# donahowe/TheaterGen

Hardware: AMD Instinct MI355X
Metric: 512px 50-step char images/sec (node), CMIGBench 4-turn story (higher is better)
Workload: dtype bf16; 1 GPU; SD-1.5 512x512, 4-turn story x 2 characters = 8 char images per step per GPU, 50 DDIM steps, CFG 7.5, IP-Adapter 77+4 tokens scale 0.4, bf16, random-init weights; plan=sd15, char_batch=8, cfg_batch=16, streams=1, ddim_steps=50, parallelism=dialogue-sharded x1 (RCCL broadcast + all_gather only)

## Files before the change

theatergen_amd/build.py:

```python
import hashlib
import os
import subprocess
import sys
from concurrent.futures import ThreadPoolExecutor

HERE = os.path.dirname(os.path.abspath(__file__))
CSRC = os.path.join(HERE, "csrc")
OBJ = os.path.join(CSRC, "_build")
LIBDIR = os.path.join(HERE, "lib")
LIB = os.path.join(LIBDIR, "libtheatergen_hip.so")
HEADER = os.path.join(os.path.dirname(HERE), "include", "theatergen_hip.h")
ARCH = "gfx950"
FLAGS = ["--offload-arch=" + ARCH, "-O3", "-std=c++17", "-fPIC",
         "-Wno-unused-result"]


EXTRA_FLAGS = {"tg_rowchain.hip": ["-mllvm", "-pragma-unroll-threshold=1000000"]}

BUILD_INFO = os.path.join(LIBDIR, "build_info.json")


def _write_build_info():
    import json

    def git(*a):
        try:
            return subprocess.run(["git", "-C", HERE] + list(a), capture_output=True, text=True).stdout.strip()
        except OSError:
            return ""
    info = {"commit": git("rev-parse", "--short", "HEAD"), "csrc_dirty": bool(git("status", "--porcelain", "--", CSRC, HEADER)),
            "sources_sha256": _digest(sources() + sorted(os.path.join(CSRC, f) for f in os.listdir(CSRC) if f.endswith(".h")) + [HEADER])[:16]}
    with open(BUILD_INFO, "w") as f:
        json.dump(info, f)


def _hipcc():
    for c in (os.environ.get("HIPCC"), "/opt/rocm/bin/hipcc", "hipcc"):
        if c and (os.path.isabs(c) and os.path.exists(c) or not os.path.isabs(c)):
            return c
    return "hipcc"


def _digest(paths):
    h = hashlib.sha256()
    for p in paths:
        with open(p, "rb") as f:
            h.update(f.read())
    h.update(" ".join(FLAGS).encode())
    for p_ in paths:
        h.update(" ".join(EXTRA_FLAGS.get(os.path.basename(p_), [])).encode())
    return h.hexdigest()


def sources():
    return sorted(os.path.join(CSRC, f) for f in os.listdir(CSRC) if f.endswith(".hip"))


def build(force=False, verbose=True, check_gate=False):
    os.makedirs(OBJ, exist_ok=True)
    os.makedirs(LIBDIR, exist_ok=True)
    srcs = sources()
    deps = [os.path.join(CSRC, f) for f in os.listdir(CSRC) if f.endswith(".h")] + [HEADER]
    hipcc = _hipcc()
    todo = []
    objs = []
    for s in srcs:
        o = os.path.join(OBJ, os.path.basename(s)[:-4] + ".o")
        stamp = o + ".sha"
        dg = _digest([s] + deps)
        objs.append(o)
        if force or not os.path.exists(o) or not os.path.exists(o + ".res") or not os.path.exists(stamp) or open(stamp).read() != dg:
            todo.append((s, o, stamp, dg))

    def compile_one(job):
        s, o, stamp, dg = job
        cmd = [hipcc] + FLAGS + EXTRA_FLAGS.get(os.path.basename(s), []) + ["-Rpass-analysis=kernel-resource-usage", "-c", s, "-o", o]
        if verbose:
            print("[build]", " ".join(cmd), flush=True)
        r = subprocess.run(cmd, capture_output=True, text=True)
        if r.returncode != 0:
            raise RuntimeError(f"hipcc failed for {s}:\n{r.stdout}\n{r.stderr}")
        with open(o + ".res", "w") as f:
            f.write(r.stderr)
        with open(stamp, "w") as f:
            f.write(dg)

    if todo:
        with ThreadPoolExecutor(max_workers=min(8, len(todo))) as ex:
            list(ex.map(compile_one, todo))
    if todo or not os.path.exists(LIB):
        cmd = [hipcc, "--offload-arch=" + ARCH, "-shared", "-fPIC", "-o", LIB] + objs
        if verbose:
            print("[build]", " ".join(cmd), flush=True)
        r = subprocess.run(cmd, capture_output=True, text=True)
        if r.returncode != 0:
            raise RuntimeError(f"link failed:\n{r.stdout}\n{r.stderr}")
    if todo or not os.path.exists(BUILD_INFO):
        _write_build_info()
    if check_gate or os.environ.get("TG_BUILD_GATE") == "1":
        write_resources(check=True, verbose=verbose, report=False)
    return LIB


RESOURCES_JSON = os.path.join(os.path.dirname(HERE), "profiles", "r6_kernel_resources.json")
HOT_GATES = [
    ("attention_kernel<bf16,48,64,true,true,false,false>", 0, 128),
    ("attention_kernel<f16,48,64,true,true,false,false>", 0, 128),
    ("attention_kernel<", 0, 256),
    ("gemm_glds_kernel<", 0, 256),
    ("conv_halo_kernel<", 0, 256),
    ("conv_slab_kernel<", 320, 256),
    ("bt_gemm_kernel<", 132, 256),
    ("rc_xattn_kernel<", 0, 256),
    ("rc_ff_kernel<", 0, 256),
    ("rc_front_kernel<", 0, 216),
    ("rc_linear_kernel<", 0, 256),
    ("skinny_gemm_kernel<", 0, 256),
    ("attn_bwd_kernel<", 0, 224),
    ("pp_gemm_kernel<bf16,2,", 0, 256),
    ("pp_gemm_kernel<f16,2,", 0, 256),
    ("pp_gemm_kernel<bf16,0,0>", 0, 256),
    ("pp_gemm_kernel<f16,0,0>", 0, 256),
    ("pp_gemm_kernel<", 256, 256),
    ("conv_in_mfma_kernel<", 0, 256),
    ("conv_out_mfma_kernel<", 0, 128),
]


def _pretty(sym):
    import re
    m = re.match(r"_ZN12_GLOBAL__N_1(\d+)", sym) or re.match(r"_Z(\d+)", sym)
    if not m:
        return sym
    n = int(m.group(1))
    base, rest = sym[m.end():m.end() + n], sym[m.end() + n:]
    if not rest.startswith("I"):
        return base
    args, i = [], 1
    while i < len(rest) and rest[i] != "E":
        if rest.startswith("DF16b", i):
            args.append("bf16"); i += 5
        elif rest.startswith("DF16_", i):
            args.append("f16"); i += 5
        elif rest[i] == "L":
            j = rest.index("E", i)
            tok = rest[i + 1:j]
            if tok[0] == "b":
                args.append("true" if tok[1:] == "1" else "false")
            else:
                args.append(re.sub(r"^[a-z]n?", lambda mm: "-" if mm.group(0).endswith("n") and len(mm.group(0)) > 1 else "", tok))
            i = j + 1
        elif rest[i] in "fidjlmb":
            args.append({"f": "float", "i": "int", "d": "double", "j": "unsigned", "l": "long", "m": "unsigned long", "b": "bool"}[rest[i]]); i += 1
        else:
            args.append("?" + rest[i:i + 12]); break
    return base + "<" + ",".join(args) + ">"


def _demangle(names):
    return [_pretty(n) for n in names]


def kernel_resources(verbose=True):
    import re
    keys = {"VGPRs": "vgprs", "AGPRs": "agprs", "ScratchSize [bytes/lane]": "scratch", "Occupancy [waves/SIMD]": "occupancy",
            "SGPRs Spill": "sgpr_spill", "VGPRs Spill": "vgpr_spill", "SGPRs": "sgprs"}
    all_recs = []
    for src in sources():
        path = os.path.join(OBJ, os.path.basename(src)[:-4] + ".o.res")
        if not os.path.exists(path):
            raise RuntimeError(f"{path} is missing: run build() first")
        cur = None
        for line in open(path).read().splitlines():
            m = re.search(r"remark: Function Name: (\S+)", line)
            if m:
                cur = {"symbol": m.group(1), "file": os.path.basename(src)}
                all_recs.append(cur)
                continue
            m = re.search(r"remark:\s+([A-Za-z][A-Za-z \[\]/]*): (\d+)", line)
            if m and cur is not None and m.group(1).strip() in keys:
                cur[keys[m.group(1).strip()]] = int(m.group(2))
    names = _demangle([r["symbol"] for r in all_recs])
    out = {}
    for r, n in zip(all_recs, names):
        r = dict(r)
        if n in out:
            n = n + " " + r["symbol"]
        out[n] = r
    if verbose:
        print(f"[resources] {len(out)} kernels", flush=True)
    return out


def check_resources(res):
    bad = []
    hits = [0] * len(HOT_GATES)
    for name, r in res.items():
        for gi, (sub, max_scratch, max_vgpr) in enumerate(HOT_GATES):
            if sub in name:
                hits[gi] += 1
                if r.get("scratch", 0) > max_scratch or r.get("vgprs", 0) > max_vgpr:
                    bad.append(f"{name}: {r.get('vgprs')} VGPRs (<= {max_vgpr}), scratch {r.get('scratch')} B (<= {max_scratch})")
                break
    for (sub, _, _), n in zip(HOT_GATES, hits):
        if n == 0:
            bad.append(f"gate '{sub}' matches no kernel")
    return bad


ASM_MFMA_KERNELS = {"tg_conv_slab_pp.o": "conv_slab_pp_kernel"}


def check_mfma_loops(verbose=True):
    import re
    import tempfile
    llvm = os.path.join(os.path.dirname(os.path.realpath(_hipcc())), "..", "lib", "llvm", "bin")
    if not os.path.exists(os.path.join(llvm, "llvm-objdump")):
        llvm = "/opt/rocm/lib/llvm/bin"
    bad = []

    def regs(tok):
        m = re.match(r"v\[(\d+):(\d+)\]", tok)
        if m:
            return set(range(int(m.group(1)), int(m.group(2)) + 1))
        m = re.match(r"v(\d+)$", tok)
        return {int(m.group(1))} if m else set()

    for obj, sub in ASM_MFMA_KERNELS.items():
        o = os.path.join(OBJ, obj)
        if not os.path.exists(o):
            continue
        with tempfile.TemporaryDirectory(prefix="tg_isa_") as td:
            fb, co = os.path.join(td, "k.fatbin"), os.path.join(td, "k.co")
            subprocess.run([os.path.join(llvm, "llvm-objcopy"), "--dump-section", ".hip_fatbin=" + fb, o], check=True)
            subprocess.run([os.path.join(llvm, "clang-offload-bundler"), "--unbundle", "--type=o", "--input=" + fb,
                            "--targets=hipv4-amdgcn-amd-amdhsa--" + ARCH, "--output=" + co], check=True)
            dis = subprocess.run([os.path.join(llvm, "llvm-objdump"), "-d", "--no-show-raw-insn", co], capture_output=True, text=True, check=True).stdout
        kern, body, kernels = None, [], []
        for line in dis.split("\n"):
            m = re.match(r"^[0-9a-f]+ <(.*)>:$", line)
            if m:
                if kern is not None:
                    kernels.append((kern, body))
                kern, body = m.group(1), []
            elif kern is not None:
                body.append(line.split("//")[0].strip())
        if kern is not None:
            kernels.append((kern, body))
        seen = 0
        for name, body in kernels:
            if sub not in name:
                continue
            mf = [i for i, t in enumerate(body) if t.startswith("v_mfma")]
            if not mf:
                continue
            seen += 1
            loop = body[mf[0]:mf[-1] + 1]
            accs = set()
            for t in loop:
                if t.startswith("v_mfma"):
                    accs |= regs(t.split(None, 1)[1].split(",")[0].strip())
            hits = [t for t in loop if t and not t.startswith("v_mfma") and any(regs(x) & accs for x in re.findall(r"v\[\d+:\d+\]|v\d+", t))]
            if hits:
                bad.append(f"{_pretty(name)}: {len(hits)} instruction(s) inside the inline-asm MFMA loop touch an accumulator register, e.g. `{hits[0]}`")
        if verbose:
            print(f"[mfma-loops] {obj}: {seen} kernels checked", flush=True)
        if seen == 0:
            bad.append(f"{obj}: no kernel matching {sub!r} with MFMAs found (the check would be vacuous)")
    return bad


def write_resources(check=False, verbose=True, report=True):
    import json
    res = kernel_resources(verbose=verbose)
    if report:
        try:
            commit = subprocess.run(["git", "rev-parse", "--short", "HEAD"], capture_output=True, text=True, cwd=HERE).stdout.strip()
        except OSError:
            commit = ""
        try:
            os.makedirs(os.path.dirname(RESOURCES_JSON), exist_ok=True)
            with open(RESOURCES_JSON, "w") as f:
                json.dump({"flags": FLAGS, "built_from_commit_or_later": commit, "gates": HOT_GATES, "kernels": dict(sorted(res.items()))}, f, indent=1)
        except OSError as e:
            print(f"[resources] cannot write {RESOURCES_JSON}: {e}", flush=True)
    bad = check_resources(res) + check_mfma_loops(verbose=verbose)
    for b in bad:
        print("[resources] GATE:", b, flush=True)
    if check and bad:
        raise RuntimeError("kernel resource gate failed:\n" + "\n".join(bad))
    return res


if __name__ == "__main__":
    if "--resources" in sys.argv:
        build()
        write_resources(check="--check" in sys.argv)
        print(RESOURCES_JSON)
    else:
        print(build(force="--force" in sys.argv))
```

theatergen_amd/csrc/tg_attention.hip:

```cpp
#include "tg_common.h"

namespace {

constexpr int KV = 64;

__device__ __attribute__((aligned(256))) unsigned char attn_zero_page[256];
#define TG_R8(x) x, x, x, x, x, x, x, x
__device__ __attribute__((aligned(256))) const unsigned short attn_ones_bf16[64] = {TG_R8(TG_R8(0x3F80))};
__device__ __attribute__((aligned(256))) const unsigned short attn_ones_f16[64] = {TG_R8(TG_R8(0x3C00))};
__device__ __attribute__((aligned(256))) const unsigned short attn_one0_bf16[8] = {0x3F80, 0, 0, 0, 0, 0, 0, 0};
__device__ __attribute__((aligned(256))) const unsigned short attn_one0_f16[8] = {0x3C00, 0, 0, 0, 0, 0, 0, 0};
template <typename T> __device__ __forceinline__ const T* one0_page();
template <> __device__ __forceinline__ const bf16_t* one0_page<bf16_t>() { return reinterpret_cast<const bf16_t*>(attn_one0_bf16); }
template <> __device__ __forceinline__ const f16_t* one0_page<f16_t>() { return reinterpret_cast<const f16_t*>(attn_one0_f16); }
template <typename T> __device__ __forceinline__ const T* ones_page();
template <> __device__ __forceinline__ const bf16_t* ones_page<bf16_t>() { return reinterpret_cast<const bf16_t*>(attn_ones_bf16); }
template <> __device__ __forceinline__ const f16_t* ones_page<f16_t>() { return reinterpret_cast<const f16_t*>(attn_ones_f16); }

struct AttnParams {
  int heads, hd, n_q, n_qblk;
  const void* q; long q_ld, q_bs;
  const void* k0; long k0_ld, k0_bs;
  const void* vt0; long vt0_ld, vt0_bs;
  int len0;
  const void* k1; long k1_ld, k1_bs;
  const void* vt1; long vt1_ld, vt1_bs;
  int len1;
  float scale_log2;
  float w1;
  const float* w1_dev;
  void* out; long out_ld, out_bs;
  int causal;
  const float* mask; long mask_bs, mask_hs, mask_qs;
  float inv_scale;
};

template <typename T, int DPAD, int DV, bool ONES, bool FOLD, bool PIPE, bool MASK>
__global__ __launch_bounds__(256) __attribute__((amdgpu_waves_per_eu(DV <= 64 ? 3 : (DV <= 96 ? 2 : 1)))) void attention_kernel(AttnParams p) {
  typedef typename Vec<T>::v8 V8;
  typedef typename Vec<T>::v4 V4;
  constexpr int NP = (DPAD + 63) / 64;
  constexpr int NKS = DPAD / 16;
  constexpr int DT = DV / 32;
  constexpr int KJ = NP * 2;
  constexpr int VJ = DV / 32;
  constexpr int K_ELEMS = NP * 64 * 64;
  constexpr int STAGE = K_ELEMS + DV * 64;

  extern __shared__ __attribute__((aligned(16))) char smem[];
  T* sbase = reinterpret_cast<T*>(smem);

  const int tid = threadIdx.x, lane = tid & 63, hi = lane >> 5, l31 = lane & 31;
  const int wave = __builtin_amdgcn_readfirstlane(tid >> 6);
  int lbid;
  {
    const int nb = gridDim.x, q8 = nb >> 3, r8 = nb & 7, xcd = blockIdx.x & 7;
    lbid = (xcd < r8 ? xcd * (q8 + 1) : r8 * (q8 + 1) + (xcd - r8) * q8) + (blockIdx.x >> 3);
  }
  const int qblk = lbid % p.n_qblk;
  const int h = (lbid / p.n_qblk) % p.heads, b = lbid / (p.n_qblk * p.heads);
  const int HD = p.hd;
  const long qrow = (long)qblk * 128 + wave * 32 + l31;
  const bool q_ok = qrow < p.n_q;

  V8 qf[NKS];
  {
    const T* qp = reinterpret_cast<const T*>(p.q) + (long)b * p.q_bs + qrow * p.q_ld + (long)h * HD;
#pragma unroll
    for (int ks = 0; ks < NKS; ++ks) {
      const int d = ks * 16 + hi * 8;
      V8 v;
#pragma unroll
      for (int j = 0; j < 8; ++j) v[j] = from_f32<T>(0.f);
      if (q_ok && d < HD) v = *reinterpret_cast<const V8*>(qp + d);
      if constexpr (FOLD) {
#pragma unroll
        for (int j = 0; j < 8; ++j) v[j] = from_f32<T>(to_f32<T>(v[j]) * p.scale_log2);
      }
      qf[ks] = v;
    }
  }
  float qbias = 0.f;

  f32x16 o[DT];
#pragma unroll
  for (int t = 0; t < DT; ++t)
#pragma unroll
    for (int r = 0; r < 16; ++r) o[t][r] = 0.f;
  float m_run = -INFINITY, l_run = 0.f;

  const int lrow = lane >> 3, slot = lane & 7;
  const T* zero = reinterpret_cast<const T*>(attn_zero_page);
  auto dma = [&](const T* src, T* lds_row_base) {
    __builtin_amdgcn_global_load_lds((const __attribute__((address_space(1))) void*)src,
                                     (__attribute__((address_space(3))) void*)lds_row_base, 16, 0, 0);
  };
  auto issue = [&](const T* kb, long k_ld, const T* vb, long vt_ld, int len, int kv0, int stage) {
    T* sK = sbase + stage * STAGE;
    T* sV = sK + K_ELEMS;
#pragma unroll
    for (int j = 0; j < KJ; ++j) {
      const int q = j * 4 + wave;
      const int prow = 8 * q + lrow;
      const int r = prow & 63, panel = prow >> 6;
      const int d0 = panel * 64 + ((slot ^ ((r >> 1) & 7)) << 3);
      const bool ok = d0 < HD && kv0 + r < len;
      const T* src = ok ? kb + (long)(kv0 + r) * k_ld + d0 : zero;
      if (FOLD && d0 == HD) src = one0_page<T>();
      dma(src, sK + q * 512);
    }
#pragma unroll
    for (int j = 0; j < VJ; ++j) {
      const int q = j * 4 + wave;
      const int d = 8 * q + lrow;
      const int c0 = kv0 + ((slot ^ ((d >> 1) & 7)) << 3);
      const T* src = (d < HD && c0 < len) ? vb + (long)d * vt_ld + c0 : zero;
      if (ONES && d == DV - 1) src = ones_page<T>();
      dma(src, sV + q * 512);
    }
  };
  auto fixup_v = [&](int rem, int stage) {
    T* sV = sbase + stage * STAGE + K_ELEMS;
    if (tid < DV && tid < HD) {
      const int d = tid, ch = rem >> 3;
      T* rowp = sV + d * 64 + ((ch ^ ((d >> 1) & 7)) << 3);
      for (int c = rem & 7; c < 8; ++c) rowp[c] = from_f32<T>(0.f);
    }
  };

  const int skey = (l31 >> 1) & 7;
  const int prow = (l31 & 19) | ((l31 & 4) << 1) | ((l31 & 8) >> 1);
  const int pkey = (prow >> 1) & 7;
  int kofs[4], vofs[4];
#pragma unroll
  for (int c = 0; c < 4; ++c) kofs[c] = prow * 64 + (((2 * c + hi) ^ pkey) << 3);
#pragma unroll
  for (int c = 0; c < 4; ++c) vofs[c] = l31 * 64 + (((2 * c + hi) ^ skey) << 3);
  auto scores = [&](f32x16 (&s)[2], const T* sK, int len, int kv0, bool causal) {
#pragma unroll
    for (int kvt = 0; kvt < 2; ++kvt) {
#pragma unroll
      for (int r = 0; r < 16; ++r) s[kvt][r] = 0.f;
#pragma unroll
      for (int ks = 0; ks < NKS; ++ks) {
        V8 kf = *reinterpret_cast<const V8*>(sK + kofs[ks & 3] + ((ks >> 2) * 4096 + kvt * 32 * 64));
        s[kvt] = mfma32(kf, qf[ks], s[kvt]);
      }
    }
    if (kv0 + KV > len || causal) {
      const int qmax = causal ? (int)qrow : 0x7fffffff;
#pragma unroll
      for (int kvt = 0; kvt < 2; ++kvt)
#pragma unroll
        for (int r = 0; r < 16; ++r) {
          const int kv = kv0 + kvt * 32 + 16 * (r >> 3) + 8 * hi + (r & 7);
          if (kv >= len || kv > qmax) s[kvt][r] = -INFINITY;
        }
    }
  };

  auto tile_max = [&](const f32x16 (&s)[2]) {
    float mx = -INFINITY;
#pragma unroll
    for (int kvt = 0; kvt < 2; ++kvt)
#pragma unroll
      for (int r = 0; r < 16; ++r) mx = fmaxf(mx, s[kvt][r]);
    float a = mx, b = mx;
    asm volatile("s_nop 1\n\tv_permlane32_swap_b32 %0, %1" : "+v"(a), "+v"(b));
    return fmaxf(a, b);
  };

  auto pv = [&](const f32x16 (&s)[2], const T* sV) {
#pragma unroll
    for (int c = 0; c < 4; ++c) {
      const int kvt = c >> 1, cc = c & 1;
      V8 pf;
#pragma unroll
      for (int j = 0; j < 8; ++j) pf[j] = from_f32<T>(s[kvt][8 * cc + j]);
#pragma unroll
      for (int t = 0; t < DT; ++t) {
        const V8 vf = *reinterpret_cast<const V8*>(sV + vofs[c] + t * 32 * 64);
        o[t] = mfma32(vf, pf, o[t]);
      }
    }
  };

  const T* kb0 = reinterpret_cast<const T*>(p.k0) + (long)b * p.k0_bs + (long)h * HD;
  const T* vb0 = reinterpret_cast<const T*>(p.vt0) + (long)b * p.vt0_bs + (long)h * HD * p.vt0_ld;
  const T* kb1 = reinterpret_cast<const T*>(p.k1) + (long)b * p.k1_bs + (long)h * HD;
  const T* vb1 = reinterpret_cast<const T*>(p.vt1) + (long)b * p.vt1_bs + (long)h * HD * p.vt1_ld;

  const int nt0 = (p.len0 + KV - 1) / KV;
  issue(kb0, p.k0_ld, vb0, p.vt0_ld, p.len0, 0, 0);
  for (int t = 0; t < nt0; ++t) {
    const int st = t & 1, kv0 = t * KV;
    asm volatile("s_waitcnt vmcnt(0)" ::: "memory");
    __builtin_amdgcn_s_barrier();
    if (kv0 + KV > p.len0 && ((p.len0 - kv0) & 7)) {
      fixup_v(p.len0 - kv0, st);
      __syncthreads();
    }
    if (t + 1 < nt0) issue(kb0, p.k0_ld, vb0, p.vt0_ld, p.len0, kv0 + KV, st ^ 1);
    else if (p.len1 > 0) issue(kb1, p.k1_ld, vb1, p.vt1_ld, p.len1, 0, st ^ 1);
    const T* sK = sbase + st * STAGE;
    f32x16 s[2];
    static_assert(!PIPE || (DV == 64 && NKS <= 3), "PIPE: head dim 40 only");
    const bool piped = PIPE && !(kv0 + KV > p.len0 || p.causal != 0);
    float tm;
    if (piped) {
      V8 kf0[NKS], kf1[NKS];
#pragma unroll
      for (int ks = 0; ks < NKS; ++ks) {
        kf0[ks] = *reinterpret_cast<const V8*>(sK + kofs[ks & 3] + (ks >> 2) * 4096);
        kf1[ks] = *reinterpret_cast<const V8*>(sK + kofs[ks & 3] + ((ks >> 2) * 4096 + 32 * 64));
      }
#pragma unroll
      for (int r = 0; r < 16; ++r) { s[0][r] = 0.f; s[1][r] = 0.f; }
      float mx = -INFINITY;
#pragma unroll
      for (int ks = 0; ks < NKS; ++ks) s[0] = mfma32(kf0[ks], qf[ks], s[0]);
      __builtin_amdgcn_sched_barrier(0);
#pragma unroll
      for (int ks = 0; ks < NKS; ++ks) {
        s[1] = mfma32(kf1[ks], qf[ks], s[1]);
#pragma unroll
        for (int r = ks * 16 / NKS; r < (ks + 1) * 16 / NKS; ++r) mx = fmaxf(mx, s[0][r]);
        __builtin_amdgcn_sched_barrier(0);
      }
#pragma unroll
      for (int r = 0; r < 16; ++r) mx = fmaxf(mx, s[1][r]);
      float a = mx, b2 = mx;
      asm volatile("s_nop 1\n\tv_permlane32_swap_b32 %0, %1" : "+v"(a), "+v"(b2));
      tm = fmaxf(a, b2);
    } else {
      scores(s, sK, p.len0, kv0, p.causal != 0);
      if constexpr (MASK) {
        const float* mp = p.mask + (long)b * p.mask_bs + (long)h * p.mask_hs + (q_ok ? qrow : 0) * p.mask_qs;
#pragma unroll
        for (int kvt = 0; kvt < 2; ++kvt)
#pragma unroll
          for (int r = 0; r < 16; ++r) {
            const int kv = kv0 + kvt * 32 + 16 * (r >> 3) + 8 * hi + (r & 7);
            if (kv < p.len0) s[kvt][r] += mp[kv] * p.inv_scale;
          }
      }
      tm = tile_max(s);
    }
    constexpr float LAZY_LOG2 = 8.f;
    float ps = 0.f;
    float mc = 0.f;
    if constexpr (FOLD) {
      if (t == 0 || __any(tm > LAZY_LOG2)) {
        const float sh = t == 0 ? tm : fmaxf(tm, 0.f);
        const float nb = to_f32<T>(from_f32<T>(qbias - sh));
        const float delta = nb - qbias;
        const float alpha = t == 0 ? 1.0f : __builtin_amdgcn_exp2f(delta);
#pragma unroll
        for (int t2 = 0; t2 < DT; ++t2)
#pragma unroll
          for (int r = 0; r < 16; ++r) o[t2][r] *= alpha;
        if (!ONES) l_run *= alpha;
#pragma unroll
        for (int kvt = 0; kvt < 2; ++kvt)
#pragma unroll
          for (int r = 0; r < 16; ++r) s[kvt][r] += delta;
        qbias = nb;
        if (hi) qf[NKS - 1][0] = from_f32<T>(nb);
      }
    } else {
      if (__any(tm * p.scale_log2 > m_run * p.scale_log2 + LAZY_LOG2)) {
        const float m_new = fmaxf(m_run, tm);
        const float alpha = __builtin_amdgcn_exp2f((m_run - m_new) * p.scale_log2);
#pragma unroll
        for (int t2 = 0; t2 < DT; ++t2)
#pragma unroll
          for (int r = 0; r < 16; ++r) o[t2][r] *= alpha;
        if (!ONES) l_run *= alpha;
        m_run = m_new;
      }
      mc = m_run * p.scale_log2;
    }
    auto ex = [&](float x) { return FOLD ? __builtin_amdgcn_exp2f(x) : __builtin_amdgcn_exp2f(__builtin_fmaf(x, p.scale_log2, -mc)); };
    const T* sV = sK + K_ELEMS;
    if (piped) {
      V8 vf[2][DT];
#pragma unroll
      for (int c = 0; c < 2; ++c)
#pragma unroll
        for (int t2 = 0; t2 < DT; ++t2) vf[c][t2] = *reinterpret_cast<const V8*>(sV + vofs[c] + t2 * 32 * 64);
#pragma unroll
      for (int r = 0; r < 16; ++r) {
        const float e = ex(s[0][r]);
        s[0][r] = e;
        if (!ONES) ps += e;
      }
      __builtin_amdgcn_sched_barrier(0);
      constexpr int EPM = 16 / (2 * DT);
#pragma unroll
      for (int c = 0; c < 2; ++c) {
        V8 pf;
#pragma unroll
        for (int j = 0; j < 8; ++j) pf[j] = from_f32<T>(s[0][8 * c + j]);
#pragma unroll
        for (int t2 = 0; t2 < DT; ++t2) {
          o[t2] = mfma32(vf[c][t2], pf, o[t2]);
#pragma unroll
          for (int r = (c * DT + t2) * EPM; r < (c * DT + t2 + 1) * EPM; ++r) {
            const float e = ex(s[1][r]);
            s[1][r] = e;
            if (!ONES) ps += e;
          }
          __builtin_amdgcn_sched_barrier(0);
        }
      }
#pragma unroll
      for (int c = 2; c < 4; ++c) {
        V8 pf;
#pragma unroll
        for (int j = 0; j < 8; ++j) pf[j] = from_f32<T>(s[1][8 * (c & 1) + j]);
#pragma unroll
        for (int t2 = 0; t2 < DT; ++t2) {
          const V8 vf2 = *reinterpret_cast<const V8*>(sV + vofs[c] + t2 * 32 * 64);
          o[t2] = mfma32(vf2, pf, o[t2]);
        }
      }
      if (!ONES) l_run += ps;
    } else {
#pragma unroll
      for (int kvt = 0; kvt < 2; ++kvt)
#pragma unroll
        for (int r = 0; r < 16; ++r) {
          const float e = ex(s[kvt][r]);
          s[kvt][r] = e;
          if (!ONES) ps += e;
        }
      if (!ONES) l_run += ps;
      pv(s, sV);
    }
  }
  {
    float l_tot;
    if (ONES) {
      const float c = hi ? o[DT - 1][15] : 0.f;
      l_tot = c + __shfl_xor(c, 32, 64);
    } else {
      l_tot = l_run + __shfl_xor(l_run, 32, 64);
    }
    const float inv = 1.f / l_tot;
#pragma unroll
    for (int t2 = 0; t2 < DT; ++t2)
#pragma unroll
      for (int r = 0; r < 16; ++r) o[t2][r] *= inv;
  }

  if (p.len1 > 0) {
    const int st = nt0 & 1;
    asm volatile("s_waitcnt vmcnt(0)" ::: "memory");
    __builtin_amdgcn_s_barrier();
    if (p.len1 < KV && (p.len1 & 7)) {
      fixup_v(p.len1, st);
      __syncthreads();
    }
    const T* sK = sbase + st * STAGE;
    f32x16 s[2];
    if constexpr (FOLD) {
      if (hi) qf[NKS - 1][0] = from_f32<T>(0.f);
    }
    scores(s, sK, p.len1, 0, false);
    const float sc1 = FOLD ? 1.0f : p.scale_log2;
    const float mc1 = tile_max(s) * sc1;
    float ps = 0.f;
#pragma unroll
    for (int kvt = 0; kvt < 2; ++kvt)
#pragma unroll
      for (int r = 0; r < 16; ++r) {
        const float e = __builtin_amdgcn_exp2f(__builtin_fmaf(s[kvt][r], sc1, -mc1));
        s[kvt][r] = e;
        ps += e;
      }
    const float l1 = ps + __shfl_xor(ps, 32, 64);
    const float f = (p.w1_dev != nullptr ? *p.w1_dev : p.w1) / l1;
#pragma unroll
    for (int kvt = 0; kvt < 2; ++kvt)
#pragma unroll
      for (int r = 0; r < 16; ++r) s[kvt][r] *= f;
    pv(s, sK + K_ELEMS);
  }

  if (q_ok) {
    T* op = reinterpret_cast<T*>(p.out) + (long)b * p.out_bs + qrow * p.out_ld + (long)h * HD;
#pragma unroll
    for (int t = 0; t < DT; ++t)
#pragma unroll
      for (int g = 0; g < 4; ++g) {
        const int d = t * 32 + 8 * g + 4 * hi;
        if (d < HD) {
          V4 v;
#pragma unroll
          for (int j = 0; j < 4; ++j) v[j] = from_f32<T>(o[t][4 * g + j]);
          *reinterpret_cast<V4*>(op + d) = v;
        }
      }
  }
}

template <typename T, int DPAD, int DV, bool ONES, bool FOLD = false, bool PIPE = false, bool MASK = false>
int launch_attn(const tg_attn_desc* d, const AttnParams& p, hipStream_t st) {
  constexpr int NP = (DPAD + 63) / 64;
  const size_t lds = (size_t)2 * (NP * 64 * 64 + DV * 64) * sizeof(T);
  AttnParams pp = p;
  pp.n_qblk = (d->n_q + 127) / 128;
  dim3 grid((unsigned)(pp.n_qblk * d->heads * d->batch));
  auto k = attention_kernel<T, DPAD, DV, ONES, FOLD, PIPE, MASK>;
  static const hipError_t attr = hipFuncSetAttribute(reinterpret_cast<const void*>(k), hipFuncAttributeMaxDynamicSharedMemorySize, (int)lds);
  (void)attr;
  hipLaunchKernelGGL(k, grid, dim3(256), lds, st, pp);
  TG_LAUNCH_CHECK();
  return TG_OK;
}

template <typename T>
int dispatch_attn(const tg_attn_desc* d, const AttnParams& p, hipStream_t st) {
  const int hd = d->head_dim;
  if (p.mask != nullptr) {
    if (hd <= 16) return launch_attn<T, 16, 32, true, false, false, true>(d, p, st);
    if (hd <= 32) return launch_attn<T, 32, 32, false, false, false, true>(d, p, st);
    if (hd <= 48) return launch_attn<T, 48, 64, true, false, false, true>(d, p, st);
    if (hd <= 64) return launch_attn<T, 64, 64, false, false, false, true>(d, p, st);
    if (hd <= 80) return launch_attn<T, 80, 96, true, false, false, true>(d, p, st);
    if (hd <= 96) return launch_attn<T, 96, 96, false, false, false, true>(d, p, st);
    if (hd <= 128) return launch_attn<T, 128, 128, false, false, false, true>(d, p, st);
    return launch_attn<T, 160, 160, false, false, false, true>(d, p, st);
  }
  if (hd <= 16) return launch_attn<T, 16, 32, true>(d, p, st);
  if (hd <= 32) return launch_attn<T, 32, 32, false>(d, p, st);
  if (hd == 40 && !getenv("TG_ATTN_NOFOLD")) {
    static const bool pipe = getenv("TG_ATTN_PIPE") != nullptr;
    return pipe ? launch_attn<T, 48, 64, true, true, true>(d, p, st) : launch_attn<T, 48, 64, true, true>(d, p, st);
  }
  if (hd <= 48) return launch_attn<T, 48, 64, true>(d, p, st);
  if (hd <= 64) return launch_attn<T, 64, 64, false>(d, p, st);
  if (hd <= 80) return launch_attn<T, 80, 96, true>(d, p, st);
  if (hd <= 96) return launch_attn<T, 96, 96, false>(d, p, st);
  if (hd <= 128) return launch_attn<T, 128, 128, false>(d, p, st);
  return launch_attn<T, 160, 160, false>(d, p, st);
}

template <typename T>
__global__ __launch_bounds__(256) void attn_probs_kernel(int b0, int heads, int hd, int n_q, const T* q, long q_ld, long q_bs,
                                                         const T* k, long k_ld, long k_bs, int len, float scale,
                                                         const int* tokens, int n_tokens, float* probs) {
  typedef typename Vec<T>::v8 V8;
  const int lane = threadIdx.x & 63;
  const long qi = (long)blockIdx.x * 4 + (threadIdx.x >> 6);
  const int h = blockIdx.y, bb = blockIdx.z, b = b0 + bb;
  if (qi >= n_q) return;
  const T* qp = q + (long)b * q_bs + qi * q_ld + (long)h * hd;
  const T* kp = k + (long)b * k_bs + (long)h * hd;
  constexpr int MAXJ = 4;
  float sc[MAXJ];
#pragma unroll
  for (int jj = 0; jj < MAXJ; ++jj) {
    const int j = lane + 64 * jj;
    float acc = 0.f;
    if (j < len) {
      for (int d = 0; d < hd; d += 8) {
        V8 a = *reinterpret_cast<const V8*>(qp + d);
        V8 c = *reinterpret_cast<const V8*>(kp + (long)j * k_ld + d);
#pragma unroll
        for (int e = 0; e < 8; ++e) acc += to_f32<T>(a[e]) * to_f32<T>(c[e]);
      }
    }
    sc[jj] = j < len ? acc * scale : -INFINITY;
  }
  float mx = -INFINITY;
#pragma unroll
  for (int jj = 0; jj < MAXJ; ++jj) mx = fmaxf(mx, sc[jj]);
  mx = wave_max(mx);
  float sum = 0.f;
#pragma unroll
  for (int jj = 0; jj < MAXJ; ++jj) { sc[jj] = __expf(sc[jj] - mx); sum += sc[jj]; }
  sum = wave_sum(sum);
  const float inv = 1.f / sum;
  const int nt = tokens ? n_tokens : len;
  float* op = probs + (((long)bb * heads + h) * n_q + qi) * nt;
  if (!tokens) {
#pragma unroll
    for (int jj = 0; jj < MAXJ; ++jj) {
      const int j = lane + 64 * jj;
      if (j < len) op[j] = sc[jj] * inv;
    }
  } else {
    for (int t = 0; t < n_tokens; ++t) {
      const int j = tokens[t];
      const int owner = j & 63, slot = j >> 6;
      float v = 0.f;
#pragma unroll
      for (int jj = 0; jj < MAXJ; ++jj)
        if (jj == slot) v = sc[jj];
      v = __shfl(v, owner, 64);
      if (lane == 0) op[t] = v * inv;
    }
  }
}

}

extern "C" int tg_attention(const tg_attn_desc* d, void* stream) {
  TG_CHECK(d != nullptr, TG_ERR_ARG, "tg_attention: null descriptor");
  TG_CHECK(d->dtype == TG_BF16 || d->dtype == TG_F16, TG_ERR_ARG, "tg_attention: bad dtype");
  TG_CHECK(d->batch > 0 && d->heads > 0 && d->n_q > 0 && d->len0 > 0, TG_ERR_ARG, "tg_attention: empty problem");
  TG_CHECK(d->head_dim > 0 && d->head_dim % 8 == 0 && d->head_dim <= 160, TG_ERR_ARG,
           "tg_attention: head_dim %d unsupported (multiple of 8, <= 160)", d->head_dim);
  TG_CHECK(d->q && d->k0 && d->vt0 && d->out, TG_ERR_ARG, "tg_attention: null q/k0/vt0/out");
  TG_CHECK(d->q_ld % 8 == 0 && d->k0_ld % 8 == 0 && d->vt0_ld % 8 == 0 && d->out_ld % 4 == 0, TG_ERR_ARG,
           "tg_attention: pitches must keep 16-byte alignment");
  TG_CHECK(d->len1 >= 0 && d->len1 <= KV, TG_ERR_ARG, "tg_attention: len1 (%d) must be <= 64", d->len1);
  if (d->len1 > 0) TG_CHECK(d->k1 && d->vt1 && d->k1_ld % 8 == 0 && d->vt1_ld % 8 == 0, TG_ERR_ARG, "tg_attention: bad segment 1");
  AttnParams p{};
  p.heads = d->heads; p.hd = d->head_dim; p.n_q = d->n_q;
  p.q = d->q; p.q_ld = d->q_ld; p.q_bs = d->q_bs;
  p.k0 = d->k0; p.k0_ld = d->k0_ld; p.k0_bs = d->k0_bs; p.vt0 = d->vt0; p.vt0_ld = d->vt0_ld; p.vt0_bs = d->vt0_bs; p.len0 = d->len0;
  p.k1 = d->k1; p.k1_ld = d->k1_ld; p.k1_bs = d->k1_bs; p.vt1 = d->vt1; p.vt1_ld = d->vt1_ld; p.vt1_bs = d->vt1_bs; p.len1 = d->len1;
  p.scale_log2 = d->scale * 1.4426950408889634f;
  p.w1 = d->w1;
  p.w1_dev = d->w1_dev;
  p.out = d->out; p.out_ld = d->out_ld; p.out_bs = d->out_bs;
  p.causal = d->causal;
  if (d->mask != nullptr) {
    TG_CHECK(d->scale > 0.f, TG_ERR_ARG, "tg_attention: an additive mask needs scale > 0");
    p.mask = d->mask; p.mask_bs = d->mask_bs; p.mask_hs = d->mask_hs; p.mask_qs = d->mask_qs;
    p.inv_scale = 1.0f / d->scale;
  }
  hipStream_t st = reinterpret_cast<hipStream_t>(stream);
  if (d->dtype == TG_BF16) return dispatch_attn<bf16_t>(d, p, st);
  return dispatch_attn<f16_t>(d, p, st);
}

extern "C" int tg_attn_probs(int32_t dtype, int32_t batch, int32_t b0, int32_t heads, int32_t head_dim, int32_t n_q,
                             const void* q, int64_t q_ld, int64_t q_bs, const void* k, int64_t k_ld, int64_t k_bs,
                             int32_t len, float scale, const int32_t* tokens, int32_t n_tokens, float* probs, void* stream) {
  TG_CHECK(dtype == TG_BF16 || dtype == TG_F16, TG_ERR_ARG, "tg_attn_probs: bad dtype");
  TG_CHECK(q && k && probs && batch > b0 && b0 >= 0 && heads > 0 && n_q > 0, TG_ERR_ARG, "tg_attn_probs: bad args");
  TG_CHECK(len > 0 && len <= 256 && head_dim % 8 == 0, TG_ERR_ARG, "tg_attn_probs: len (%d) must be in 1..256", len);
  hipStream_t st = reinterpret_cast<hipStream_t>(stream);
  dim3 grid((unsigned)((n_q + 3) / 4), (unsigned)heads, (unsigned)(batch - b0));
  if (dtype == TG_BF16)
    hipLaunchKernelGGL(attn_probs_kernel<bf16_t>, grid, dim3(256), 0, st, b0, heads, head_dim, n_q, (const bf16_t*)q, q_ld, q_bs,
                       (const bf16_t*)k, k_ld, k_bs, len, scale, tokens, n_tokens, probs);
  else
    hipLaunchKernelGGL(attn_probs_kernel<f16_t>, grid, dim3(256), 0, st, b0, heads, head_dim, n_q, (const f16_t*)q, q_ld, q_bs,
                       (const f16_t*)k, k_ld, k_bs, len, scale, tokens, n_tokens, probs);
  TG_LAUNCH_CHECK();
  return TG_OK;
}
```

Baseline: 9.490 char_images/s.

## Add ping-pong 512-thread attention kernel for head_dim 40 small-grid cases

Adds a new flash-attention kernel for head_dim 40 that uses 8 waves over 256 query rows, a 4-stage global_load_lds K/V ring, and two staggered wave groups with priority and barrier offsets so that the QK and PV MFMA phases of one group overlap softmax work in the other. Lazy rescaling skips the output rescale unless the running max grows past a threshold. It is used by default when the grid is at most 256 blocks, there is a single unmasked, non-causal KV segment that is a multiple of 64, and the output is aligned. The goal is to fill the GPU better and hide latency on small attention grids. In exchange it adds a large, intricate kernel with tight synchronisation and only narrow applicability.

```diff
diff --git a/theatergen_amd/build.py b/theatergen_amd/build.py
--- a/theatergen_amd/build.py
+++ b/theatergen_amd/build.py
@@ -107,6 +107,8 @@
     ("attention_kernel<bf16,48,64,true,true,false,false>", 0, 128),
     ("attention_kernel<f16,48,64,true,true,false,false>", 0, 128),
     ("attention_kernel<", 0, 256),
+    ("attention_pp_kernel<bf16>", 0, 168),
+    ("attention_pp_kernel<f16>", 0, 168),
     ("gemm_glds_kernel<", 0, 256),
     ("conv_halo_kernel<", 0, 256),
     ("conv_slab_kernel<", 320, 256),
diff --git a/theatergen_amd/csrc/tg_attention.hip b/theatergen_amd/csrc/tg_attention.hip
--- a/theatergen_amd/csrc/tg_attention.hip
+++ b/theatergen_amd/csrc/tg_attention.hip
@@ -404,6 +404,235 @@
   }
 }
 
+constexpr int PP_STAGES = 4;
+constexpr int PP_STAGE_ELEMS = 64 * 64 + 64 * 64;
+constexpr long PP_MAX_GRID = 256;
+
+template <typename T>
+__global__ __launch_bounds__(512) void attention_pp_kernel(AttnParams p) {
+  typedef typename Vec<T>::v8 V8;
+  typedef typename Vec<T>::v4 V4;
+  constexpr int NKS = 3, DT = 2, K_ELEMS = 64 * 64;
+  extern __shared__ __attribute__((aligned(16))) char smem[];
+  T* sbase = reinterpret_cast<T*>(smem);
+
+  const int tid = threadIdx.x, lane = tid & 63, hi = lane >> 5, l31 = lane & 31;
+  const int wave = __builtin_amdgcn_readfirstlane(tid >> 6);
+  const bool lag = wave >= 4;
+  int lbid;
+  {
+    const int nb = gridDim.x, q8 = nb >> 3, r8 = nb & 7, xcd = blockIdx.x & 7;
+    lbid = (xcd < r8 ? xcd * (q8 + 1) : r8 * (q8 + 1) + (xcd - r8) * q8) + (blockIdx.x >> 3);
+  }
+  const int qblk = lbid % p.n_qblk;
+  const int h = (lbid / p.n_qblk) % p.heads, b = lbid / (p.n_qblk * p.heads);
+  const int HD = p.hd;
+  const long qrow = (long)qblk * 256 + wave * 32 + l31;
+  const bool q_ok = qrow < p.n_q;
+
+  V8 qf[NKS];
+  {
+    const T* qp = reinterpret_cast<const T*>(p.q) + (long)b * p.q_bs + qrow * p.q_ld + (long)h * HD;
+#pragma unroll
+    for (int ks = 0; ks < NKS; ++ks) {
+      const int d = ks * 16 + hi * 8;
+      V8 v;
+#pragma unroll
+      for (int j = 0; j < 8; ++j) v[j] = from_f32<T>(0.f);
+      if (q_ok && d < HD) v = *reinterpret_cast<const V8*>(qp + d);
+#pragma unroll
+      for (int j = 0; j < 8; ++j) v[j] = from_f32<T>(to_f32<T>(v[j]) * p.scale_log2);
+      qf[ks] = v;
+    }
+  }
+  float qbias = 0.f;
+
+  f32x16 o[DT];
+#pragma unroll
+  for (int t = 0; t < DT; ++t)
+#pragma unroll
+    for (int r = 0; r < 16; ++r) o[t][r] = 0.f;
+
+  const int lrow = lane >> 3, slot = lane & 7;
+  const T* kb = reinterpret_cast<const T*>(p.k0) + (long)b * p.k0_bs + (long)h * HD;
+  const T* vb = reinterpret_cast<const T*>(p.vt0) + (long)b * p.vt0_bs + (long)h * HD * p.vt0_ld;
+  const T* zero = reinterpret_cast<const T*>(attn_zero_page);
+  const int r8 = 8 * wave + lrow;
+  const int kd0 = (slot ^ ((r8 >> 1) & 7)) << 3;
+  const T* ksrc = kd0 < HD ? kb + (long)r8 * p.k0_ld + kd0 : (kd0 == HD ? one0_page<T>() : zero);
+  const long kstep = kd0 < HD ? (long)KV * p.k0_ld : 0;
+  const T* vsrc = r8 < HD ? vb + (long)r8 * p.vt0_ld + ((slot ^ ((r8 >> 1) & 7)) << 3) : (r8 == 63 ? ones_page<T>() : zero);
+  const int vstep = r8 < HD ? KV : 0;
+  auto issue = [&](int t) {
+    T* sK = sbase + (t & (PP_STAGES - 1)) * PP_STAGE_ELEMS;
+    __builtin_amdgcn_global_load_lds((const __attribute__((address_space(1))) void*)(ksrc + t * kstep),
+                                     (__attribute__((address_space(3))) void*)(sK + wave * 512), 16, 0, 0);
+    __builtin_amdgcn_global_load_lds((const __attribute__((address_space(1))) void*)(vsrc + t * vstep),
+                                     (__attribute__((address_space(3))) void*)(sK + K_ELEMS + wave * 512), 16, 0, 0);
+  };
+
+  const int skey = (l31 >> 1) & 7;
+  const int prow = (l31 & 19) | ((l31 & 4) << 1) | ((l31 & 8) >> 1);
+  const int pkey = (prow >> 1) & 7;
+  int kofs[NKS], vofs[4];
+#pragma unroll
+  for (int c = 0; c < NKS; ++c) kofs[c] = prow * 64 + (((2 * c + hi) ^ pkey) << 3);
+#pragma unroll
+  for (int c = 0; c < 4; ++c) vofs[c] = l31 * 64 + (((2 * c + hi) ^ skey) << 3);
+
+  const int nt = p.len0 / KV;
+  issue(0);
+  if (nt > 1) {
+    issue(1);
+    asm volatile("s_waitcnt vmcnt(2)" ::: "memory");
+  } else {
+    asm volatile("s_waitcnt vmcnt(0)" ::: "memory");
+  }
+  __builtin_amdgcn_s_barrier();
+  if (__builtin_amdgcn_readfirstlane(tid) >= 256) __builtin_amdgcn_s_setprio(1);
+  if (lag) __builtin_amdgcn_s_barrier();
+
+  f32x16 s[2];
+  V8 pf[4];
+  for (int t = 0;; ++t) {
+    {
+      const T* sK = sbase + (t & (PP_STAGES - 1)) * PP_STAGE_ELEMS;
+      const T* sV = sbase + ((t - 1) & (PP_STAGES - 1)) * PP_STAGE_ELEMS + K_ELEMS;
+      auto rd = [](const T* a) { return *reinterpret_cast<const V8*>(a); };
+      V8 kf[NKS];
+      if (t > 0) {
+        V8 va[2][DT], vb2[2][DT];
+#pragma unroll
+        for (int c = 0; c < 2; ++c)
+#pragma unroll
+          for (int t2 = 0; t2 < DT; ++t2) va[c][t2] = rd(sV + vofs[c] + t2 * 32 * 64);
+        __builtin_amdgcn_sched_barrier(0);
+#pragma unroll
+        for (int c = 0; c < 2; ++c)
+#pragma unroll
+          for (int t2 = 0; t2 < DT; ++t2) vb2[c][t2] = rd(sV + vofs[2 + c] + t2 * 32 * 64);
+#pragma unroll
+        for (int c = 0; c < 2; ++c)
+#pragma unroll
+          for (int t2 = 0; t2 < DT; ++t2) o[t2] = mfma32(va[c][t2], pf[c], o[t2]);
+        __builtin_amdgcn_sched_barrier(0);
+        if (t < nt) {
+#pragma unroll
+          for (int ks = 0; ks < NKS; ++ks) kf[ks] = rd(sK + kofs[ks]);
+        }
+#pragma unroll
+        for (int c = 0; c < 2; ++c)
+#pragma unroll
+          for (int t2 = 0; t2 < DT; ++t2) o[t2] = mfma32(vb2[c][t2], pf[2 + c], o[t2]);
+        __builtin_amdgcn_sched_barrier(0);
+      } else {
+#pragma unroll
+        for (int ks = 0; ks < NKS; ++ks) kf[ks] = rd(sK + kofs[ks]);
+      }
+      if (t == nt) break;
+      V8 kf1[NKS];
+#pragma unroll
+      for (int ks = 0; ks < NKS; ++ks) kf1[ks] = rd(sK + kofs[ks] + 32 * 64);
+#pragma unroll
+      for (int r = 0; r < 16; ++r) s[0][r] = 0.f;
+#pragma unroll
+      for (int ks = 0; ks < NKS; ++ks) s[0] = mfma32(kf[ks], qf[ks], s[0]);
+      __builtin_amdgcn_sched_barrier(0);
+#pragma unroll
+      for (int r = 0; r < 16; ++r) s[1][r] = 0.f;
+#pragma unroll
+      for (int ks = 0; ks < NKS; ++ks) s[1] = mfma32(kf1[ks], qf[ks], s[1]);
+    }
+    if (lag) asm volatile("s_waitcnt vmcnt(0)" ::: "memory");
+    __builtin_amdgcn_s_barrier();
+
+    const bool more = t + 2 < nt;
+    if (more) issue(t + 2);
+    float tm;
+    {
+      float mx = -INFINITY;
+#pragma unroll
+      for (int kvt = 0; kvt < 2; ++kvt)
+#pragma unroll
+        for (int r = 0; r < 16; ++r) mx = fmaxf(mx, s[kvt][r]);
+      float a = mx, c = mx;
+      asm volatile("s_nop 1\n\tv_permlane32_swap_b32 %0, %1" : "+v"(a), "+v"(c));
+      tm = fmaxf(a, c);
+    }
+    constexpr float LAZY_LOG2 = 8.f;
+    if (t == 0 || __any(tm > LAZY_LOG2)) {
+      const float sh = t == 0 ? tm : fmaxf(tm, 0.f);
+      const float nb = to_f32<T>(from_f32<T>(qbias - sh));
+      const float delta = nb - qbias;
+      const float alpha = t == 0 ? 1.0f : __builtin_amdgcn_exp2f(delta);
+#pragma unroll
+      for (int t2 = 0; t2 < DT; ++t2)
+#pragma unroll
+        for (int r = 0; r < 16; ++r) o[t2][r] *= alpha;
+#pragma unroll
+      for (int kvt = 0; kvt < 2; ++kvt)
+#pragma unroll
+        for (int r = 0; r < 16; ++r) s[kvt][r] += delta;
+      qbias = nb;
+      if (hi) qf[NKS - 1][0] = from_f32<T>(nb);
+    }
+#pragma unroll
+    for (int c = 0; c < 4; ++c)
+#pragma unroll
+      for (int j = 0; j < 8; ++j) pf[c][j] = from_f32<T>(__builtin_amdgcn_exp2f(s[c >> 1][8 * (c & 1) + j]));
+    if (!lag) {
+      if (more) asm volatile("s_waitcnt vmcnt(2)" ::: "memory");
+      else asm volatile("s_waitcnt vmcnt(0)" ::: "memory");
+    }
+    __builtin_amdgcn_s_barrier();
+  }
+  if (!lag) __builtin_amdgcn_s_barrier();
+
+  {
+    const float c = hi ? o[DT - 1][15] : 0.f;
+    const float l_tot = c + __shfl_xor(c, 32, 64);
+    const float inv = 1.f / l_tot;
+#pragma unroll
+    for (int t2 = 0; t2 < DT; ++t2)
+#pragma unroll
+      for (int r = 0; r < 16; ++r) o[t2][r] *= inv;
+    asm volatile("" : "+v"(o[0]), "+v"(o[1]));
+  }
+  if (q_ok) {
+    T* op = reinterpret_cast<T*>(p.out) + (long)b * p.out_bs + qrow * p.out_ld + (long)h * HD;
+    u32x2 w[6];
+#pragma unroll
+    for (int g = 0; g < 5; ++g) {
+      V4 v;
+#pragma unroll
+      for (int j = 0; j < 4; ++j) v[j] = from_f32<T>(o[g >> 2][4 * (g & 3) + j]);
+      w[g] = __builtin_bit_cast(u32x2, v);
+    }
+    w[5] = u32x2{0u, 0u};
+#pragma unroll
+    for (int k = 0; k < 6; k += 2) {
+      unsigned a0 = w[k][0], b0 = w[k + 1][0], a1 = w[k][1], b1 = w[k + 1][1];
+      asm volatile("s_nop 1\n\tv_permlane32_swap_b32 %0, %1" : "+v"(a0), "+v"(b0));
+      asm volatile("s_nop 1\n\tv_permlane32_swap_b32 %0, %1" : "+v"(a1), "+v"(b1));
+      if (k < 4 || !hi) *reinterpret_cast<u32x4*>(op + 8 * k + 8 * hi) = u32x4{a0, a1, b0, b1};
+    }
+  }
+}
+
+template <typename T>
+int launch_attn_pp(const tg_attn_desc* d, const AttnParams& p, hipStream_t st) {
+  const size_t lds = (size_t)PP_STAGES * PP_STAGE_ELEMS * sizeof(T);
+  AttnParams pp = p;
+  pp.n_qblk = (d->n_q + 255) / 256;
+  dim3 grid((unsigned)(pp.n_qblk * d->heads * d->batch));
+  auto k = attention_pp_kernel<T>;
+  static const hipError_t attr = hipFuncSetAttribute(reinterpret_cast<const void*>(k), hipFuncAttributeMaxDynamicSharedMemorySize, (int)lds);
+  (void)attr;
+  hipLaunchKernelGGL(k, grid, dim3(512), lds, st, pp);
+  TG_LAUNCH_CHECK();
+  return TG_OK;
+}
+
 template <typename T, int DPAD, int DV, bool ONES, bool FOLD = false, bool PIPE = false, bool MASK = false>
 int launch_attn(const tg_attn_desc* d, const AttnParams& p, hipStream_t st) {
   constexpr int NP = (DPAD + 63) / 64;
@@ -435,6 +664,12 @@
   if (hd <= 16) return launch_attn<T, 16, 32, true>(d, p, st);
   if (hd <= 32) return launch_attn<T, 32, 32, false>(d, p, st);
   if (hd == 40 && !getenv("TG_ATTN_NOFOLD")) {
+    const char* pp_env = getenv("TG_ATTN_PP");
+    const char pp_mode = pp_env ? pp_env[0] : '1';
+    const long pp_grid = (long)((d->n_q + 255) / 256) * d->heads * d->batch;
+    if (pp_mode != '0' && p.len1 == 0 && p.causal == 0 && p.len0 % KV == 0 && d->out_ld % 8 == 0 && d->out_bs % 8 == 0 &&
+        (reinterpret_cast<uintptr_t>(d->out) & 15) == 0 && (pp_mode == '2' || pp_grid <= PP_MAX_GRID))
+      return launch_attn_pp<T>(d, p, st);
     static const bool pipe = getenv("TG_ATTN_PIPE") != nullptr;
     return pipe ? launch_attn<T, 48, 64, true, true, true>(d, p, st) : launch_attn<T, 48, 64, true, true>(d, p, st);
   }
```

Result: no change. 9.501 char_images/s, median of 3 (+0.1%).
